# uber/petastorm

Measured on AMD Instinct MI355X. Metric: samples/sec/node (make_batch_reader->PyTorch DataLoader), imagenet config, higher is better.
Workload: dtype fp32; 1 GPU; model=ImageNetSchema(224x224x3 jpeg CompressedImageCodec + int32 label), global_batch=256, parallelism=dp1, prime_batches=0

## Files before the change

petastorm_amd/gpu/decoder.py:

```python

import os

import numpy as np
import torch

from petastorm_amd import ops
from petastorm_amd.codecs import (CompressedImageCodec, NdarrayCodec)

_ENC_PLAIN = 0
_ENC_PLAIN_DICT = 2
_ENC_RLE = 3
_ENC_DELTA_BINARY = 5
_ENC_DELTA_LENGTH_BA = 6
_ENC_DELTA_BA = 7
_ENC_RLE_DICT = 8
_ENC_BYTE_STREAM_SPLIT = 9
_PAGE_DATA_V1 = 0
_PAGE_DICT = 2
_PAGE_DATA_V2 = 3

_PHYS_TO_TORCH = {
    'INT32': (torch.int32, 4),
    'INT64': (torch.int64, 8),
    'FLOAT': (torch.float32, 4),
# ... 1268 lines not shown
                          status)
        self._check(status, 'png-inflate:' + field.name)
        out_bytes = row_bytes * heights
        out_off = np.zeros(n, dtype=np.int64)
        out_off[1:] = np.cumsum(out_bytes)[:-1]
        out = torch.empty(int(out_bytes.sum()) + _SLACK, dtype=torch.uint8,
                          device=dev)
        st2 = self._status(n)
        ext.png_unfilter_batch(raw, self._up(raw_off), out,
                               self._up(out_off),
                               self._up(meta['height']),
                               self._up(meta['row_bytes']),
                               self._up(meta['bpp']), st2)
        self._check(st2, 'png-unfilter:' + field.name)
        if len(set(widths.tolist())) != 1 or len(set(heights.tolist())) != 1 \
                or len(set(channels.tolist())) != 1 \
                or len(set(depth.tolist())) != 1:
            return None
        h, w, c, d = int(heights[0]), int(widths[0]), int(channels[0]), \
            int(depth[0])
        out = out[:int(out_bytes.sum())]
        if d == 16:
            ext.bswap16(out)
            t = out.view(torch.int16).view(n, h, w, c)
            t = t.to(torch.int32) & 0xFFFF
        else:
            t = out.view(n, h, w, c)
        return t.squeeze(-1) if c == 1 else t

    def decode_jpeg_column(self, col, field, fused_norm=None):
        if col.host_buf is None:
            return None
        ext = self._ext
        dev = self.device
        meta = col.jpeg_meta
        if meta is None:
            host_off = torch.from_numpy(col.host_val_off)
            host_len = col.val_len.cpu()
            meta = ext.jpeg_parse_batch(col.host_buf, host_off, host_len)
        n = col.n
        widths = meta['width'].numpy()
        heights = meta['height'].numpy()
        ncomp = meta['ncomp'].numpy()
        meta_dev = {}
        for k, v in meta.items():
            if not isinstance(v, torch.Tensor):
                meta_dev[k] = v
            elif k in ('seg_pos', 'seg_end'):
                meta_dev[k] = self._up(v)
            else:
                meta_dev[k] = self._up_cached(v)
        block_total = int(meta['block_total'])
        samp_total = int(meta['samp_total'])
        coef = torch.zeros(block_total * 64, dtype=torch.float32, device=dev)
        samples = torch.empty(samp_total, dtype=torch.uint8, device=dev)
        n_segs = int(meta['seg_img'].numel())
        uniform = (len(set(widths.tolist())) == 1 and
                   len(set(heights.tolist())) == 1 and
                   len(set(ncomp.tolist())) == 1)
        if fused_norm is not None and uniform and \
                self.device.type == 'cuda':
            H, W = int(heights[0]), int(widths[0])
            out_px = (widths.astype(np.int64) * heights * 3)
            out_off = np.zeros(n, dtype=np.int64)
            out_off[1:] = np.cumsum(out_px)[:-1]
            out = torch.empty(n, 3, H, W, dtype=torch.float32, device=dev)
            cache = getattr(self, '_fused_norm_cache', None)
            if cache is None:
                cache = self._fused_norm_cache = {}
            key = (tuple(fused_norm.mean), tuple(fused_norm.std))
            if key not in cache:
                mean_t = torch.tensor(fused_norm.mean, dtype=torch.float32,
                                      device=dev)
                inv_t = 1.0 / torch.tensor(fused_norm.std,
                                           dtype=torch.float32, device=dev)
                cache[key] = (mean_t, inv_t)
            mean_t, inv_t = cache[key]
            status = self._status(max(n_segs, 1))
            ext.jpeg_decode_fused_batch(
                col.device_buf, meta_dev, coef, samples, out.view(-1),
                self._up_cached(torch.from_numpy(out_off)), mean_t, inv_t,
                1.0 / fused_norm.scale_div, status)
            self._check(status, 'jpeg-fused:' + field.name)
            return out
        out_bytes = (widths.astype(np.int64) * heights *
                     np.where(ncomp == 3, 3, 1))
        out_off = np.zeros(n, dtype=np.int64)
        out_off[1:] = np.cumsum(out_bytes)[:-1]
        out = torch.empty(int(out_bytes.sum()), dtype=torch.uint8,
                          device=dev)
        status = self._status(max(n_segs, 1))
        ext.jpeg_decode_batch(col.device_buf, meta_dev, coef, samples, out,
                              self._up_cached(torch.from_numpy(out_off)),
                              status)
        self._check(status, 'jpeg:' + field.name)
        if uniform:
            c = 3 if ncomp[0] == 3 else 1
            t = out.view(n, int(heights[0]), int(widths[0]), c)
            return t if c == 3 else t.squeeze(-1)
        return None


def _widen_unsigned(t, np_dtype):
    if np_dtype == np.dtype(np.uint16):
        return t.to(torch.int32) & 0xFFFF
    if np_dtype == np.dtype(np.uint32):
        return t.to(torch.int64) & 0xFFFFFFFF
# ... 17 lines not shown
```

petastorm_amd/ops/csrc/ext.cpp:

```cpp
#include <torch/extension.h>

namespace psa {

void snappy_decompress_batch(torch::Tensor comp, torch::Tensor comp_start,
                             torch::Tensor comp_end, torch::Tensor out,
                             torch::Tensor out_offsets,
                             torch::Tensor out_len, torch::Tensor status);
void lz4_decompress_batch(torch::Tensor comp, torch::Tensor blk_start,
                          torch::Tensor blk_end, torch::Tensor out,
                          torch::Tensor out_offsets, torch::Tensor out_len,
                          torch::Tensor status);

void zstd_decompress_host(torch::Tensor src, torch::Tensor src_off,
                          torch::Tensor src_len, torch::Tensor dst,
                          torch::Tensor dst_off, torch::Tensor dst_len,
                          torch::Tensor status);

int64_t zstd_work_bytes();
void zstd_decompress_batch(torch::Tensor src, torch::Tensor src_off,
                           torch::Tensor src_len, torch::Tensor dst,
                           torch::Tensor dst_off, torch::Tensor dst_len,
                           torch::Tensor work, torch::Tensor status);

void rle_hybrid_decode_batch(torch::Tensor data, torch::Tensor start,
                             torch::Tensor end, torch::Tensor bit_width,
                             torch::Tensor n_values, torch::Tensor out_off,
                             torch::Tensor out, torch::Tensor status);
void byte_array_offsets_batch(torch::Tensor data, torch::Tensor start,
                              torch::Tensor end, torch::Tensor n_values,
                              torch::Tensor out_off, torch::Tensor val_off,
                              torch::Tensor val_len, torch::Tensor status);
void varlen_gather(torch::Tensor src, torch::Tensor src_off,
                   torch::Tensor lengths, torch::Tensor dst,
                   torch::Tensor dst_off);
void plain_fixed_decode_batch(torch::Tensor page_buf,
                              torch::Tensor payload_start,
                              torch::Tensor payload_end,
                              torch::Tensor n_values, torch::Tensor row0,
                              int64_t def_mode, int64_t esize,
                              int64_t fill_pattern, torch::Tensor def_buf,
                              torch::Tensor def_start, torch::Tensor def_len,
                              torch::Tensor out,
                              torch::Tensor valid_out, torch::Tensor status);
void npy_payload_offsets(torch::Tensor data, torch::Tensor val_off,
                         torch::Tensor val_len, torch::Tensor pay_off,
                         torch::Tensor pay_len, torch::Tensor status);
void nhwc_to_nchw_normalize(torch::Tensor in, torch::Tensor out,
                            torch::Tensor mean, torch::Tensor inv_std,
                            double scale);
py::dict jpeg_parse_batch(torch::Tensor buf, torch::Tensor val_off,
                          torch::Tensor val_len);
py::dict parquet_walk_pages(torch::Tensor buf, torch::Tensor chunk_off,
                            torch::Tensor chunk_len);
void inflate_batch(torch::Tensor src, torch::Tensor seg_off,
                   torch::Tensor seg_len, torch::Tensor seg_first,
                   torch::Tensor seg_count, torch::Tensor dst,
                   torch::Tensor dst_off, torch::Tensor dst_cap,
                   torch::Tensor produced, int64_t mode,
                   torch::Tensor status);
void png_unfilter_batch(torch::Tensor raw, torch::Tensor raw_off,
                        torch::Tensor out, torch::Tensor out_off,
                        torch::Tensor height, torch::Tensor row_bytes,
                        torch::Tensor bpp, torch::Tensor status);
void bswap16(torch::Tensor data);
py::dict png_parse_batch(torch::Tensor buf, torch::Tensor val_off,
                         torch::Tensor val_len);
py::dict byte_array_host_offsets(torch::Tensor buf, torch::Tensor val_start,
                                 torch::Tensor counts);
void jpeg_decode_batch(torch::Tensor data, py::dict meta, torch::Tensor coef,
                       torch::Tensor samples, torch::Tensor out,
                       torch::Tensor out_off, torch::Tensor status);
void delta_binary_packed_batch(torch::Tensor page_buf, torch::Tensor start,
                               torch::Tensor end, torch::Tensor n_values,
                               torch::Tensor out_off, torch::Tensor out,
                               int64_t esize, torch::Tensor status);
void delta_length_byte_array_batch(torch::Tensor page_buf,
                                   torch::Tensor start, torch::Tensor end,
                                   torch::Tensor n_values,
                                   torch::Tensor out_idx,
                                   torch::Tensor val_off,
                                   torch::Tensor val_len,
                                   torch::Tensor status);
void delta_byte_array_lengths_batch(torch::Tensor page_buf,
                                    torch::Tensor start, torch::Tensor end,
                                    torch::Tensor n_values,
                                    torch::Tensor out_idx,
                                    torch::Tensor pre, torch::Tensor sfx,
                                    torch::Tensor suf_data_pos,
                                    torch::Tensor status);
void delta_byte_array_reconstruct_batch(
    torch::Tensor page_buf, torch::Tensor n_values, torch::Tensor out_idx,
    torch::Tensor pre, torch::Tensor sfx, torch::Tensor suf_data_pos,
    torch::Tensor val_off, torch::Tensor out, torch::Tensor status);
void byte_stream_split_batch(torch::Tensor page_buf, torch::Tensor start,
                             torch::Tensor n_values, torch::Tensor out_off,
                             torch::Tensor out, int64_t esize);
void bool_unpack_batch(torch::Tensor page_buf, torch::Tensor start,
                       torch::Tensor n_values, torch::Tensor out_off,
                       torch::Tensor out);
void jpeg_decode_fused_batch(torch::Tensor data, py::dict meta,
                             torch::Tensor coef, torch::Tensor samples,
                             torch::Tensor out, torch::Tensor out_off,
                             torch::Tensor mean, torch::Tensor inv_std,
                             double scale, torch::Tensor status);

}

PYBIND11_MODULE(TORCH_EXTENSION_NAME, m) {
  m.doc() = "petastorm_amd MI355X (gfx950) decode kernels";
  m.def("snappy_decompress_batch", &psa::snappy_decompress_batch,
        "Batched snappy page decompression (wave-per-page)");
  m.def("lz4_decompress_batch", &psa::lz4_decompress_batch,
        "batch LZ4 block decompression, one wave per block");
  m.def("zstd_decompress_host", &psa::zstd_decompress_host,
        "batch ZSTD frame decompression on host threads (from-scratch "
        "RFC 8878 decoder, GIL released)");
  m.def("zstd_work_bytes", &psa::zstd_work_bytes,
        "per-frame device workspace size for zstd_decompress_batch");
  m.def("zstd_decompress_batch", &psa::zstd_decompress_batch,
        "batch ZSTD frame decompression on device (thread per frame)");
  m.def("rle_hybrid_decode_batch", &psa::rle_hybrid_decode_batch,
        "Parquet RLE/bit-packed hybrid decode (levels & dict indices)");
  m.def("byte_array_offsets_batch", &psa::byte_array_offsets_batch,
        "PLAIN byte-array page -> per-value (offset, length)");
  m.def("varlen_gather", &psa::varlen_gather,
        "Unaligned variable-length byte gather (funnel-shift copy)");
  m.def("plain_fixed_decode_batch", &psa::plain_fixed_decode_batch,
        "Fused PLAIN data-page decode: def levels + prefix scan + scatter");
  m.def("npy_payload_offsets", &psa::npy_payload_offsets,
        ".npy container -> payload (offset, length)");
  m.def("nhwc_to_nchw_normalize", &psa::nhwc_to_nchw_normalize,
        "Fused uint8 NHWC -> float NCHW normalize (LDS-tiled)");
  m.def("parquet_walk_pages", &psa::parquet_walk_pages,
        "Walk Parquet page headers (thrift compact) in a raw column chunk");
  m.def("inflate_batch", &psa::inflate_batch,
        "Batched DEFLATE inflate (zlib/raw), thread-per-stream");
  m.def("png_unfilter_batch", &psa::png_unfilter_batch,
        "PNG scanline unfilter (wave-per-image, bpp-lane chains)");
  m.def("bswap16", &psa::bswap16, "byte-swap 16-bit samples in place");
  m.def("png_parse_batch", &psa::png_parse_batch,
        "Host-side PNG container parse");
  m.def("byte_array_host_offsets", &psa::byte_array_host_offsets,
        "Host-side PLAIN byte-array offset scan");
  m.def("jpeg_parse_batch", &psa::jpeg_parse_batch,
        "Host-side JPEG header/segment parse");
  m.def("jpeg_decode_batch", &psa::jpeg_decode_batch,
        "GPU baseline JPEG decode (huffman/idct/color kernels)");
  m.def("delta_binary_packed_batch", &psa::delta_binary_packed_batch,
        "DELTA_BINARY_PACKED page decode (wave-per-page, shfl prefix scan)");
  m.def("delta_length_byte_array_batch",
        &psa::delta_length_byte_array_batch,
        "DELTA_LENGTH_BYTE_ARRAY page -> per-value (offset, length)");
  m.def("delta_byte_array_lengths_batch",
        &psa::delta_byte_array_lengths_batch,
        "DELTA_BYTE_ARRAY pass 1: prefix/suffix lengths");
  m.def("delta_byte_array_reconstruct_batch",
        &psa::delta_byte_array_reconstruct_batch,
        "DELTA_BYTE_ARRAY pass 2: materialize front-coded values");
  m.def("byte_stream_split_batch", &psa::byte_stream_split_batch,
        "BYTE_STREAM_SPLIT de-interleave");
  m.def("bool_unpack_batch", &psa::bool_unpack_batch,
        "PLAIN boolean bit-unpack");
  m.def("jpeg_decode_fused_batch", &psa::jpeg_decode_fused_batch,
        "JPEG decode with fused YCbCr->RGB + normalize + NCHW fp32 "
        "epilogue (skips the NHWC uint8 intermediate)");
}
```

petastorm_amd/ops/csrc/jpeg.hip:

```cpp
#include <hip/hip_runtime.h>
#include <torch/extension.h>
#include <c10/hip/HIPStream.h>
#include "common.h"

namespace psa {

__constant__ int ZIGZAG_NAT[64] = {
    0,  1,  8,  16, 9,  2,  3,  10, 17, 24, 32, 25, 18, 11, 4,  5,
    12, 19, 26, 33, 40, 48, 41, 34, 27, 20, 13, 6,  7,  14, 21, 28,
    35, 42, 49, 56, 57, 50, 43, 36, 29, 22, 15, 23, 30, 37, 44, 51,
    58, 59, 52, 45, 38, 31, 39, 46, 53, 60, 61, 54, 47, 55, 62, 63};

__constant__ float IDCT_B[8][8] = {
    {0.35355339f, 0.35355339f, 0.35355339f, 0.35355339f,
     0.35355339f, 0.35355339f, 0.35355339f, 0.35355339f},
    {0.49039264f, 0.41573481f, 0.27778512f, 0.09754516f,
     -0.09754516f, -0.27778512f, -0.41573481f, -0.49039264f},
    {0.46193977f, 0.19134172f, -0.19134172f, -0.46193977f,
     -0.46193977f, -0.19134172f, 0.19134172f, 0.46193977f},
    {0.41573481f, -0.09754516f, -0.49039264f, -0.27778512f,
     0.27778512f, 0.49039264f, 0.09754516f, -0.41573481f},
    {0.35355339f, -0.35355339f, -0.35355339f, 0.35355339f,
     0.35355339f, -0.35355339f, -0.35355339f, 0.35355339f},
    {0.27778512f, -0.49039264f, 0.09754516f, 0.41573481f,
     -0.41573481f, -0.09754516f, 0.49039264f, -0.27778512f},
    {0.19134172f, -0.46193977f, 0.46193977f, -0.19134172f,
     -0.19134172f, 0.46193977f, -0.46193977f, 0.19134172f},
    {0.09754516f, -0.27778512f, 0.41573481f, -0.49039264f,
     0.49039264f, -0.41573481f, 0.27778512f, -0.09754516f}};

struct JpegTables {
  const int32_t* lut;
  const int32_t* maxcode;
  const int32_t* mincode;
  const int32_t* valptr;
  const uint8_t* huffval;
  const float* qtabs;
};

struct JpegGeom {
  const int32_t* comp_h;
  const int32_t* comp_v;
  const int32_t* comp_q;
  const int32_t* comp_dc;
  const int32_t* comp_ac;
  const int64_t* samp_off;
  const int32_t* samp_stride;
  const int32_t* mcus_x;
  const int32_t* mcus_y;
  const int32_t* ncomp;
  const int32_t* width;
  const int32_t* height;
  const int64_t* img_block0;
  const int32_t* bpm;
  const int32_t* kmap;
};


struct BitReader {
  const uint8_t* p;
  int64_t pos, end;
  uint64_t buf;
  int cnt;
  uint32_t sw0, sw1;
  int64_t spos;
  int scount;

  __device__ void init(const uint8_t* data, int64_t lo, int64_t hi) {
    p = data; pos = lo; end = hi; buf = 0; cnt = 0; scount = 0; spos = 0;
  }
  __device__ __forceinline__ void fill() {
    while (cnt <= 32) {
      if (pos + 4 <= end) {
        uint32_t w;
        if (scount > 0 && spos == pos) {
          w = sw0;
          sw0 = sw1;
          spos += 4;
          --scount;
        } else {
          scount = 0;
          w = (uint32_t)p[pos] | ((uint32_t)p[pos + 1] << 8) |
              ((uint32_t)p[pos + 2] << 16) | ((uint32_t)p[pos + 3] << 24);
          if (pos + 12 <= end) {
            sw0 = (uint32_t)p[pos + 4] | ((uint32_t)p[pos + 5] << 8) |
                  ((uint32_t)p[pos + 6] << 16) |
                  ((uint32_t)p[pos + 7] << 24);
            sw1 = (uint32_t)p[pos + 8] | ((uint32_t)p[pos + 9] << 8) |
                  ((uint32_t)p[pos + 10] << 16) |
                  ((uint32_t)p[pos + 11] << 24);
            spos = pos + 4;
            scount = 2;
          } else if (pos + 8 <= end) {
            sw0 = (uint32_t)p[pos + 4] | ((uint32_t)p[pos + 5] << 8) |
                  ((uint32_t)p[pos + 6] << 16) |
                  ((uint32_t)p[pos + 7] << 24);
            spos = pos + 4;
            scount = 1;
          }
        }
        uint32_t inv = ~w;
        if (!((inv - 0x01010101u) & ~inv & 0x80808080u)) {
          uint32_t be = __builtin_bswap32(w);
          buf |= (uint64_t)be << (32 - cnt);
          cnt += 32;
          pos += 4;
          continue;
        }
      }
      uint8_t b = 0;
      if (pos < end) {
        b = p[pos];
        if (b == 0xFF) {
          if (pos + 1 < end && p[pos + 1] == 0x00) {
            pos += 2;
          } else {
            pos = end;
            b = 0;
          }
        } else {
          pos += 1;
        }
      } else {
        buf |= 0;
        cnt += 8;
        continue;
      }
      buf |= (uint64_t)b << (56 - cnt);
      cnt += 8;
    }
  }
  __device__ __forceinline__ uint32_t peek(int n) {
    return (uint32_t)(buf >> (64 - n));
  }
  __device__ __forceinline__ void consume(int n) {
    buf <<= n;
    cnt -= n;
  }
};

__device__ __forceinline__ int huff_decode(BitReader& br,
                                           const JpegTables& t, int tid) {
  br.fill();
  uint32_t look = br.peek(8);
  int32_t hit = t.lut[tid * 256 + look];
  if (hit >= 0) {
    br.consume(hit >> 16);
    return hit & 0xFF;
  }
  for (int l = 9; l <= 16; ++l) {
    int32_t code = (int32_t)br.peek(l);
    int32_t mc = t.maxcode[tid * 18 + l];
    if (mc >= 0 && code <= mc) {
      br.consume(l);
      int idx = t.valptr[tid * 18 + l] + code - t.mincode[tid * 18 + l];
      return t.huffval[tid * 256 + idx];
    }
  }
  return -1;
}

__device__ __forceinline__ int receive_extend(BitReader& br, int s) {
  br.fill();
  int v = (int)br.peek(s);
  br.consume(s);
  if (v < (1 << (s - 1))) v += (-1 << s) + 1;
  return v;
}

template <bool NT>
__device__ __forceinline__ int decode_block(BitReader& br,
                                            const JpegTables& tabs,
                                            const float* __restrict__ q,
                                            int dc_t, int ac_t,
                                            float* __restrict__ out,
                                            int& pred) {
  int t = huff_decode(br, tabs, dc_t);
  if (t < 0 || t > 15) return 10;
  int diff = t ? receive_extend(br, t) : 0;
  pred += diff;
  if (NT) __builtin_nontemporal_store((float)pred * q[0], out);
  else out[0] = (float)pred * q[0];
  int kk = 1;
  while (kk < 64) {
    int rs = huff_decode(br, tabs, ac_t);
    if (rs < 0) return 11;
    int r = rs >> 4, sz = rs & 15;
    if (sz == 0) {
      if (r != 15) break;
      kk += 16;
    } else {
      kk += r;
      if (kk > 63) return 12;
      int v = receive_extend(br, sz);
      if (NT) __builtin_nontemporal_store((float)v * q[kk],
                                          out + ZIGZAG_NAT[kk]);
      else out[ZIGZAG_NAT[kk]] = (float)v * q[kk];
      ++kk;
    }
  }
  return 0;
}

template <bool NT>
__global__ void jpeg_huffman_kernel(
    const uint8_t* __restrict__ data, JpegTables tabs, JpegGeom g,
    const int32_t* __restrict__ seg_img, const int64_t* __restrict__ seg_pos,
    const int64_t* __restrict__ seg_end, const int32_t* __restrict__ seg_mcu0,
    const int32_t* __restrict__ seg_nmcu, float* __restrict__ coef,
    int32_t* __restrict__ status, int n_segs) {
  int s = blockIdx.x * blockDim.x + threadIdx.x;
  if (s >= n_segs) return;
  const int img = seg_img[s];
  const int bpm = g.bpm[img];
  const int ncomp = g.ncomp[img];

  BitReader br;
  br.init(data, seg_pos[s], seg_end[s]);

  const float* q0 = tabs.qtabs + (int64_t)g.comp_q[img * 3 + 0] * 64;
  const int dc0 = g.comp_dc[img * 3 + 0], ac0 = g.comp_ac[img * 3 + 0];
  const int rep0 = g.comp_h[img * 3 + 0] * g.comp_v[img * 3 + 0];
  const float* q1 = q0;
  const float* q2 = q0;
  int dc1 = 0, ac1 = 0, dc2 = 0, ac2 = 0;
  if (ncomp == 3) {
    q1 = tabs.qtabs + (int64_t)g.comp_q[img * 3 + 1] * 64;
    dc1 = g.comp_dc[img * 3 + 1];
    ac1 = g.comp_ac[img * 3 + 1];
    q2 = tabs.qtabs + (int64_t)g.comp_q[img * 3 + 2] * 64;
    dc2 = g.comp_dc[img * 3 + 2];
    ac2 = g.comp_ac[img * 3 + 2];
  }

  int pred0 = 0, pred1 = 0, pred2 = 0;
  const int mcu0 = seg_mcu0[s];
  const int nmcu = seg_nmcu[s];
  const int64_t blk0 = g.img_block0[img];

  for (int m = 0; m < nmcu; ++m) {
    float* mcu_out = coef + (blk0 + (int64_t)(mcu0 + m) * bpm) * 64;
    int rc = 0;
    for (int r = 0; r < rep0 && !rc; ++r, mcu_out += 64)
      rc = decode_block<NT>(br, tabs, q0, dc0, ac0, mcu_out, pred0);
    if (!rc && ncomp == 3) {
      rc = decode_block<NT>(br, tabs, q1, dc1, ac1, mcu_out, pred1);
      mcu_out += 64;
      if (!rc)
        rc = decode_block<NT>(br, tabs, q2, dc2, ac2, mcu_out, pred2);
    }
    if (rc) { status[s] = rc; return; }
  }
}


__global__ void jpeg_idct_kernel(const float* __restrict__ coef,
                                 JpegGeom g, uint8_t* __restrict__ samples,
                                 int n_imgs, int64_t block_total) {
  int64_t b = (int64_t)blockIdx.x * blockDim.x + threadIdx.x;
  if (b >= block_total) return;
  int lo = 0, hi = n_imgs - 1;
  while (lo < hi) {
    int mid = (lo + hi + 1) >> 1;
    if (g.img_block0[mid] <= b) lo = mid; else hi = mid - 1;
  }
  const int img = lo;
  const int bpm = g.bpm[img];
  const int64_t r = b - g.img_block0[img];
  const int m = (int)(r / bpm);
  const int k = (int)(r % bpm);
  const int km = g.kmap[img * 8 + k];
  const int c = km >> 8, v = (km >> 4) & 15, h = km & 15;
  const int mx = m % g.mcus_x[img];
  const int my = m / g.mcus_x[img];
  const int stride = g.samp_stride[img * 3 + c];
  uint8_t* dst = samples + g.samp_off[img * 3 + c] +
                 ((int64_t)(my * g.comp_v[img * 3 + c] + v) * 8) * stride +
                 (int64_t)(mx * g.comp_h[img * 3 + c] + h) * 8;

  const float* C = coef + b * 64;
  float tmp[64];
#pragma unroll
  for (int vv = 0; vv < 8; ++vv) {
#pragma unroll
    for (int x = 0; x < 8; ++x) {
      float acc = 0.f;
#pragma unroll
      for (int u = 0; u < 8; ++u) acc += C[vv * 8 + u] * IDCT_B[u][x];
      tmp[vv * 8 + x] = acc;
    }
  }
#pragma unroll
  for (int y = 0; y < 8; ++y) {
    uint8_t row[8];
#pragma unroll
    for (int x = 0; x < 8; ++x) {
      float acc = 0.f;
#pragma unroll
      for (int vv = 0; vv < 8; ++vv) acc += tmp[vv * 8 + x] * IDCT_B[vv][y];
      int pix = __float2int_rn(acc) + 128;
      row[x] = (uint8_t)min(255, max(0, pix));
    }
    *(uint64_t*)(dst + (int64_t)y * stride) = *(const uint64_t*)row;
  }
// ... 147 lines not shown
      rpix[k] = ((float)min(255, max(0, rv)) * scale - m0) * s0;
      gpix[k] = ((float)min(255, max(0, gv)) * scale - m1) * s1;
      bpix[k] = ((float)min(255, max(0, bv)) * scale - m2) * s2;
    }
    float* dr = dst + pix0;
    float* dg = dst + plane + pix0;
    float* db = dst + 2 * plane + pix0;
    if (cnt == 4 && ((pix0 & 3) == 0)) {
      *(float4*)dr = make_float4(rpix[0], rpix[1], rpix[2], rpix[3]);
      *(float4*)dg = make_float4(gpix[0], gpix[1], gpix[2], gpix[3]);
      *(float4*)db = make_float4(bpix[0], bpix[1], bpix[2], bpix[3]);
    } else {
      for (int k = 0; k < cnt; ++k) {
        dr[k] = rpix[k];
        dg[k] = gpix[k];
        db[k] = bpix[k];
      }
    }
  }
}


static JpegTables make_tables(const py::dict& d) {
  JpegTables t;
  t.lut = d["lut"].cast<torch::Tensor>().data_ptr<int32_t>();
  t.maxcode = d["maxcode"].cast<torch::Tensor>().data_ptr<int32_t>();
  t.mincode = d["mincode"].cast<torch::Tensor>().data_ptr<int32_t>();
  t.valptr = d["valptr"].cast<torch::Tensor>().data_ptr<int32_t>();
  t.huffval = d["huffval"].cast<torch::Tensor>().data_ptr<uint8_t>();
  t.qtabs = d["qtabs"].cast<torch::Tensor>().data_ptr<float>();
  return t;
}

static JpegGeom make_geom(const py::dict& d) {
  JpegGeom g;
  g.comp_h = d["comp_h"].cast<torch::Tensor>().data_ptr<int32_t>();
  g.comp_v = d["comp_v"].cast<torch::Tensor>().data_ptr<int32_t>();
  g.comp_q = d["comp_q"].cast<torch::Tensor>().data_ptr<int32_t>();
  g.comp_dc = d["comp_dc"].cast<torch::Tensor>().data_ptr<int32_t>();
  g.comp_ac = d["comp_ac"].cast<torch::Tensor>().data_ptr<int32_t>();
  g.samp_off = d["samp_off"].cast<torch::Tensor>().data_ptr<int64_t>();
  g.samp_stride = d["samp_stride"].cast<torch::Tensor>().data_ptr<int32_t>();
  g.mcus_x = d["mcus_x"].cast<torch::Tensor>().data_ptr<int32_t>();
  g.mcus_y = d["mcus_y"].cast<torch::Tensor>().data_ptr<int32_t>();
  g.ncomp = d["ncomp"].cast<torch::Tensor>().data_ptr<int32_t>();
  g.width = d["width"].cast<torch::Tensor>().data_ptr<int32_t>();
  g.height = d["height"].cast<torch::Tensor>().data_ptr<int32_t>();
  g.img_block0 = d["img_block0"].cast<torch::Tensor>().data_ptr<int64_t>();
  g.bpm = d["bpm"].cast<torch::Tensor>().data_ptr<int32_t>();
  g.kmap = d["kmap"].cast<torch::Tensor>().data_ptr<int32_t>();
  return g;
}

void jpeg_decode_batch(torch::Tensor data, py::dict meta, torch::Tensor coef,
                       torch::Tensor samples, torch::Tensor out,
                       torch::Tensor out_off, torch::Tensor status) {
  TORCH_CHECK(data.is_cuda() && coef.is_cuda() && samples.is_cuda() &&
              out.is_cuda());
  JpegTables tabs = make_tables(meta);
  JpegGeom g = make_geom(meta);
  auto seg_img = meta["seg_img"].cast<torch::Tensor>();
  auto seg_pos = meta["seg_pos"].cast<torch::Tensor>();
  auto seg_end = meta["seg_end"].cast<torch::Tensor>();
  auto seg_mcu0 = meta["seg_mcu0"].cast<torch::Tensor>();
  auto seg_nmcu = meta["seg_nmcu"].cast<torch::Tensor>();
  int n_segs = (int)seg_img.numel();
  int n_imgs = (int)meta["width"].cast<torch::Tensor>().numel();
  int64_t block_total = coef.numel() / 64;
  hipStream_t stream = c10::hip::getCurrentHIPStream();

  static const bool use_nt = [] {
    const char* e = getenv("PSA_JPEG_NT");
    return e && e[0] == '1';
  }();
  if (use_nt)
    hipLaunchKernelGGL(jpeg_huffman_kernel<true>,
                       dim3((n_segs + 63) / 64), dim3(64), 0, stream,
                       data.data_ptr<uint8_t>(), tabs, g,
                       seg_img.data_ptr<int32_t>(),
                       seg_pos.data_ptr<int64_t>(),
                       seg_end.data_ptr<int64_t>(),
                       seg_mcu0.data_ptr<int32_t>(),
                       seg_nmcu.data_ptr<int32_t>(), coef.data_ptr<float>(),
                       status.data_ptr<int32_t>(), n_segs);
  else
    hipLaunchKernelGGL(jpeg_huffman_kernel<false>,
                       dim3((n_segs + 63) / 64), dim3(64), 0, stream,
                       data.data_ptr<uint8_t>(), tabs, g,
                       seg_img.data_ptr<int32_t>(),
                       seg_pos.data_ptr<int64_t>(),
                       seg_end.data_ptr<int64_t>(),
                       seg_mcu0.data_ptr<int32_t>(),
                       seg_nmcu.data_ptr<int32_t>(), coef.data_ptr<float>(),
                       status.data_ptr<int32_t>(), n_segs);

  hipLaunchKernelGGL(jpeg_idct_kernel,
                     dim3((unsigned)((block_total + 255) / 256)), dim3(256),
                     0, stream, coef.data_ptr<float>(), g,
                     samples.data_ptr<uint8_t>(), n_imgs, block_total);

  int64_t avg_bytes = n_imgs > 0 ? out.numel() / n_imgs : 0;
  int64_t est_blocks = (avg_bytes / 12 + 255) / 256;
  int grid_x = (int)std::min<int64_t>(std::max<int64_t>(est_blocks, 1), 2048);
  hipLaunchKernelGGL(jpeg_color_kernel, dim3(grid_x, n_imgs), dim3(256), 0,
                     stream, samples.data_ptr<uint8_t>(), g,
                     out.data_ptr<uint8_t>(), out_off.data_ptr<int64_t>(),
                     n_imgs);
}

void jpeg_decode_fused_batch(torch::Tensor data, py::dict meta,
                             torch::Tensor coef, torch::Tensor samples,
                             torch::Tensor out, torch::Tensor out_off,
                             torch::Tensor mean, torch::Tensor inv_std,
                             double scale, torch::Tensor status) {
  TORCH_CHECK(data.is_cuda() && coef.is_cuda() && samples.is_cuda() &&
              out.is_cuda() && out.scalar_type() == torch::kFloat32);
  TORCH_CHECK(mean.is_cuda() && inv_std.is_cuda() &&
              mean.numel() == 3 && inv_std.numel() == 3);
  JpegTables tabs = make_tables(meta);
  JpegGeom g = make_geom(meta);
  auto seg_img = meta["seg_img"].cast<torch::Tensor>();
  auto seg_pos = meta["seg_pos"].cast<torch::Tensor>();
  auto seg_end = meta["seg_end"].cast<torch::Tensor>();
  auto seg_mcu0 = meta["seg_mcu0"].cast<torch::Tensor>();
  auto seg_nmcu = meta["seg_nmcu"].cast<torch::Tensor>();
  int n_segs = (int)seg_img.numel();
  int n_imgs = (int)meta["width"].cast<torch::Tensor>().numel();
  int64_t block_total = coef.numel() / 64;
  hipStream_t stream = c10::hip::getCurrentHIPStream();

  static const bool use_nt = [] {
    const char* e = getenv("PSA_JPEG_NT");
    return e && e[0] == '1';
  }();
  if (use_nt)
    hipLaunchKernelGGL(jpeg_huffman_kernel<true>,
                       dim3((n_segs + 63) / 64), dim3(64), 0, stream,
                       data.data_ptr<uint8_t>(), tabs, g,
                       seg_img.data_ptr<int32_t>(),
                       seg_pos.data_ptr<int64_t>(),
                       seg_end.data_ptr<int64_t>(),
                       seg_mcu0.data_ptr<int32_t>(),
                       seg_nmcu.data_ptr<int32_t>(), coef.data_ptr<float>(),
                       status.data_ptr<int32_t>(), n_segs);
  else
    hipLaunchKernelGGL(jpeg_huffman_kernel<false>,
                       dim3((n_segs + 63) / 64), dim3(64), 0, stream,
                       data.data_ptr<uint8_t>(), tabs, g,
                       seg_img.data_ptr<int32_t>(),
                       seg_pos.data_ptr<int64_t>(),
                       seg_end.data_ptr<int64_t>(),
                       seg_mcu0.data_ptr<int32_t>(),
                       seg_nmcu.data_ptr<int32_t>(), coef.data_ptr<float>(),
                       status.data_ptr<int32_t>(), n_segs);

  hipLaunchKernelGGL(jpeg_idct_kernel,
                     dim3((unsigned)((block_total + 255) / 256)), dim3(256),
                     0, stream, coef.data_ptr<float>(), g,
                     samples.data_ptr<uint8_t>(), n_imgs, block_total);

  int64_t avg_px = n_imgs > 0 ? out.numel() / (3 * n_imgs) : 0;
  int64_t est_blocks = (avg_px / 4 + 255) / 256;
  int grid_x = (int)std::min<int64_t>(std::max<int64_t>(est_blocks, 1), 2048);
  hipLaunchKernelGGL(jpeg_color_norm_kernel, dim3(grid_x, n_imgs), dim3(256),
                     0, stream, samples.data_ptr<uint8_t>(), g,
                     out.data_ptr<float>(), out_off.data_ptr<int64_t>(),
                     mean.data_ptr<float>(), inv_std.data_ptr<float>(),
                     (float)scale, n_imgs);
}

}
```

Baseline: 559,900 samples/sec.

## Stage JPEG Huffman tables and bitstream in LDS with tiled coefficient stores

```diff
diff --git a/petastorm_amd/gpu/decoder.py b/petastorm_amd/gpu/decoder.py
--- a/petastorm_amd/gpu/decoder.py
+++ b/petastorm_amd/gpu/decoder.py
@@ -1344,7 +1344,7 @@
                 meta_dev[k] = self._up_cached(v)
         block_total = int(meta['block_total'])
         samp_total = int(meta['samp_total'])
-        coef = torch.zeros(block_total * 64, dtype=torch.float32, device=dev)
+        coef = torch.empty(block_total * 64, dtype=torch.float32, device=dev)
         samples = torch.empty(samp_total, dtype=torch.uint8, device=dev)
         n_segs = int(meta['seg_img'].numel())
         uniform = (len(set(widths.tolist())) == 1 and
diff --git a/petastorm_amd/ops/csrc/ext.cpp b/petastorm_amd/ops/csrc/ext.cpp
--- a/petastorm_amd/ops/csrc/ext.cpp
+++ b/petastorm_amd/ops/csrc/ext.cpp
@@ -69,7 +69,8 @@
                                  torch::Tensor counts);
 void jpeg_decode_batch(torch::Tensor data, py::dict meta, torch::Tensor coef,
                        torch::Tensor samples, torch::Tensor out,
-                       torch::Tensor out_off, torch::Tensor status);
+                       torch::Tensor out_off, torch::Tensor status,
+                       int64_t staging);
 void delta_binary_packed_batch(torch::Tensor page_buf, torch::Tensor start,
                                torch::Tensor end, torch::Tensor n_values,
                                torch::Tensor out_off, torch::Tensor out,
@@ -102,7 +103,8 @@
                              torch::Tensor coef, torch::Tensor samples,
                              torch::Tensor out, torch::Tensor out_off,
                              torch::Tensor mean, torch::Tensor inv_std,
-                             double scale, torch::Tensor status);
+                             double scale, torch::Tensor status,
+                             int64_t staging);
 
 }
 
@@ -145,7 +147,10 @@
   m.def("jpeg_parse_batch", &psa::jpeg_parse_batch,
         "Host-side JPEG header/segment parse");
   m.def("jpeg_decode_batch", &psa::jpeg_decode_batch,
-        "GPU baseline JPEG decode (huffman/idct/color kernels)");
+        "GPU baseline JPEG decode (huffman/idct/color kernels)",
+        py::arg("data"), py::arg("meta"), py::arg("coef"),
+        py::arg("samples"), py::arg("out"), py::arg("out_off"),
+        py::arg("status"), py::arg("staging") = -1);
   m.def("delta_binary_packed_batch", &psa::delta_binary_packed_batch,
         "DELTA_BINARY_PACKED page decode (wave-per-page, shfl prefix scan)");
   m.def("delta_length_byte_array_batch",
@@ -163,5 +168,9 @@
         "PLAIN boolean bit-unpack");
   m.def("jpeg_decode_fused_batch", &psa::jpeg_decode_fused_batch,
         "JPEG decode with fused YCbCr->RGB + normalize + NCHW fp32 "
-        "epilogue (skips the NHWC uint8 intermediate)");
+        "epilogue (skips the NHWC uint8 intermediate)",
+        py::arg("data"), py::arg("meta"), py::arg("coef"),
+        py::arg("samples"), py::arg("out"), py::arg("out_off"),
+        py::arg("mean"), py::arg("inv_std"), py::arg("scale"),
+        py::arg("status"), py::arg("staging") = -1);
 }
diff --git a/petastorm_amd/ops/csrc/jpeg.hip b/petastorm_amd/ops/csrc/jpeg.hip
--- a/petastorm_amd/ops/csrc/jpeg.hip
+++ b/petastorm_amd/ops/csrc/jpeg.hip
@@ -57,47 +57,82 @@
 };
 
 
+constexpr int kLdsHuff = 4;
+constexpr int kLdsQ = 4;
+constexpr int kWinBytes = 8192;
+
+typedef float f32x4 __attribute__((ext_vector_type(4)));
+
+__constant__ uint8_t NAT_ZIGZAG[64] = {
+    0,  1,  5,  6,  14, 15, 27, 28, 2,  4,  7,  13, 16, 26, 29, 42,
+    3,  8,  12, 17, 25, 30, 41, 43, 9,  11, 18, 24, 31, 40, 44, 53,
+    10, 19, 23, 32, 39, 45, 52, 54, 20, 22, 33, 38, 46, 51, 55, 60,
+    21, 34, 37, 47, 50, 56, 59, 61, 35, 36, 48, 49, 57, 58, 62, 63};
+
+struct GlobalBytes {
+  typedef int64_t pos_t;
+  static constexpr bool kPrefetch = true;
+  const uint8_t* p;
+  __device__ __forceinline__ uint32_t byte(pos_t i) const { return p[i]; }
+  __device__ __forceinline__ uint32_t word(pos_t i) const {
+    return (uint32_t)p[i] | ((uint32_t)p[i + 1] << 8) |
+           ((uint32_t)p[i + 2] << 16) | ((uint32_t)p[i + 3] << 24);
+  }
+};
+
+struct LdsBytes {
+  typedef int pos_t;
+  static constexpr bool kPrefetch = false;
+  const uint32_t* w;
+  __device__ __forceinline__ uint32_t byte(pos_t i) const {
+    return (w[i >> 2] >> ((i & 3) * 8)) & 0xFFu;
+  }
+  __device__ __forceinline__ uint32_t word(pos_t i) const {
+    const uint64_t two = ((uint64_t)w[(i >> 2) + 1] << 32) | w[i >> 2];
+    return (uint32_t)(two >> ((i & 3) * 8));
+  }
+};
+
+template <class Src>
 struct BitReader {
-  const uint8_t* p;
-  int64_t pos, end;
+  typedef typename Src::pos_t pos_t;
+  Src src;
+  pos_t pos, end;
   uint64_t buf;
   int cnt;
   uint32_t sw0, sw1;
-  int64_t spos;
+  pos_t spos;
   int scount;
 
-  __device__ void init(const uint8_t* data, int64_t lo, int64_t hi) {
-    p = data; pos = lo; end = hi; buf = 0; cnt = 0; scount = 0; spos = 0;
+  __device__ void init(Src s, pos_t lo, pos_t hi) {
+    src = s; pos = lo; end = hi; buf = 0; cnt = 0; scount = 0; spos = 0;
   }
   __device__ __forceinline__ void fill() {
     while (cnt <= 32) {
       if (pos + 4 <= end) {
         uint32_t w;
-        if (scount > 0 && spos == pos) {
-          w = sw0;
-          sw0 = sw1;
-          spos += 4;
-          --scount;
+        if constexpr (Src::kPrefetch) {
+          if (scount > 0 && spos == pos) {
+            w = sw0;
+            sw0 = sw1;
+            spos += 4;
+            --scount;
+          } else {
+            scount = 0;
+            w = src.word(pos);
+            if (pos + 12 <= end) {
+              sw0 = src.word(pos + 4);
+              sw1 = src.word(pos + 8);
+              spos = pos + 4;
+              scount = 2;
+            } else if (pos + 8 <= end) {
+              sw0 = src.word(pos + 4);
+              spos = pos + 4;
+              scount = 1;
+            }
+          }
         } else {
-          scount = 0;
-          w = (uint32_t)p[pos] | ((uint32_t)p[pos + 1] << 8) |
-              ((uint32_t)p[pos + 2] << 16) | ((uint32_t)p[pos + 3] << 24);
-          if (pos + 12 <= end) {
-            sw0 = (uint32_t)p[pos + 4] | ((uint32_t)p[pos + 5] << 8) |
-                  ((uint32_t)p[pos + 6] << 16) |
-                  ((uint32_t)p[pos + 7] << 24);
-            sw1 = (uint32_t)p[pos + 8] | ((uint32_t)p[pos + 9] << 8) |
-                  ((uint32_t)p[pos + 10] << 16) |
-                  ((uint32_t)p[pos + 11] << 24);
-            spos = pos + 4;
-            scount = 2;
-          } else if (pos + 8 <= end) {
-            sw0 = (uint32_t)p[pos + 4] | ((uint32_t)p[pos + 5] << 8) |
-                  ((uint32_t)p[pos + 6] << 16) |
-                  ((uint32_t)p[pos + 7] << 24);
-            spos = pos + 4;
-            scount = 1;
-          }
+          w = src.word(pos);
         }
         uint32_t inv = ~w;
         if (!((inv - 0x01010101u) & ~inv & 0x80808080u)) {
@@ -108,11 +143,11 @@
           continue;
         }
       }
-      uint8_t b = 0;
+      uint32_t b = 0;
       if (pos < end) {
-        b = p[pos];
+        b = src.byte(pos);
         if (b == 0xFF) {
-          if (pos + 1 < end && p[pos + 1] == 0x00) {
+          if (pos + 1 < end && src.byte(pos + 1) == 0x00) {
             pos += 2;
           } else {
             pos = end;
@@ -122,7 +157,6 @@
           pos += 1;
         }
       } else {
-        buf |= 0;
         cnt += 8;
         continue;
       }
@@ -139,15 +173,46 @@
   }
 };
 
-__device__ __forceinline__ int huff_decode(BitReader& br,
-                                           const JpegTables& t, int tid) {
+template <bool TAB>
+struct HuffTabs {
+  JpegTables t;
+  const uint16_t* lut16;
+  const int32_t* maxcode;
+  const int32_t* valoff;
+  const uint8_t* huffval;
+  const uint8_t* zz;
+};
+
+template <class Src, bool TAB>
+__device__ __forceinline__ int huff_decode(BitReader<Src>& br,
+                                           const HuffTabs<TAB>& ht, int tid) {
   br.fill();
   uint32_t look = br.peek(8);
-  int32_t hit = t.lut[tid * 256 + look];
-  if (hit >= 0) {
-    br.consume(hit >> 16);
-    return hit & 0xFF;
-  }
+  if constexpr (TAB) {
+    uint32_t e = ht.lut16[tid * 256 + look];
+    if (e != 0xFFFFu) {
+      br.consume(e >> 8);
+      return e & 0xFF;
+    }
+    const uint32_t look16 = br.peek(16);
+    int len = 0;
+#pragma unroll
+    for (int l = 16; l >= 9; --l) {
+      const int32_t mc = ht.maxcode[tid * 18 + l];
+      if (mc >= 0 && (int32_t)(look16 >> (16 - l)) <= mc) len = l;
+    }
+    if (len == 0) return -1;
+    br.consume(len);
+    const int idx = ht.valoff[tid * 18 + len] + (int)(look16 >> (16 - len));
+    return ht.huffval[tid * 256 + (idx & 255)];
+  } else {
+    int32_t hit = ht.t.lut[tid * 256 + look];
+    if (hit >= 0) {
+      br.consume(hit >> 16);
+      return hit & 0xFF;
+    }
+  }
+  const JpegTables& t = ht.t;
   for (int l = 9; l <= 16; ++l) {
     int32_t code = (int32_t)br.peek(l);
     int32_t mc = t.maxcode[tid * 18 + l];
@@ -160,30 +225,32 @@
   return -1;
 }
 
-__device__ __forceinline__ int receive_extend(BitReader& br, int s) {
-  br.fill();
+template <class Src>
+__device__ __forceinline__ int receive_extend(BitReader<Src>& br, int s) {
   int v = (int)br.peek(s);
   br.consume(s);
   if (v < (1 << (s - 1))) v += (-1 << s) + 1;
   return v;
 }
 
-template <bool NT>
-__device__ __forceinline__ int decode_block(BitReader& br,
-                                            const JpegTables& tabs,
-                                            const float* __restrict__ q,
-                                            int dc_t, int ac_t,
-                                            float* __restrict__ out,
-                                            int& pred) {
-  int t = huff_decode(br, tabs, dc_t);
+__device__ __forceinline__ int tile_swz(int b) {
+  return ((b & 15) << 2) | (((b >> 4) & 1) << 1);
+}
+
+template <class Src, bool TAB>
+__device__ __forceinline__ int decode_block(BitReader<Src>& br,
+                                            const HuffTabs<TAB>& ht,
+                                            int dc_t, int ac_t, float q_dc,
+                                            int16_t* blk, int swz,
+                                            int& pred, float& dc_out) {
+  int t = huff_decode(br, ht, dc_t);
   if (t < 0 || t > 15) return 10;
   int diff = t ? receive_extend(br, t) : 0;
   pred += diff;
-  if (NT) __builtin_nontemporal_store((float)pred * q[0], out);
-  else out[0] = (float)pred * q[0];
+  dc_out = (float)pred * q_dc;
   int kk = 1;
   while (kk < 64) {
-    int rs = huff_decode(br, tabs, ac_t);
+    int rs = huff_decode(br, ht, ac_t);
     if (rs < 0) return 11;
     int r = rs >> 4, sz = rs & 15;
     if (sz == 0) {
@@ -193,63 +260,243 @@
       kk += r;
       if (kk > 63) return 12;
       int v = receive_extend(br, sz);
-      if (NT) __builtin_nontemporal_store((float)v * q[kk],
-                                          out + ZIGZAG_NAT[kk]);
-      else out[ZIGZAG_NAT[kk]] = (float)v * q[kk];
+      int nat;
+      if constexpr (TAB) nat = ht.zz[kk];
+      else nat = ZIGZAG_NAT[kk];
+      blk[nat ^ swz] = (int16_t)v;
       ++kk;
     }
   }
   return 0;
 }
 
-template <bool NT>
-__global__ void jpeg_huffman_kernel(
-    const uint8_t* __restrict__ data, JpegTables tabs, JpegGeom g,
+template <bool TAB>
+__device__ __forceinline__ void drain_tile(uint64_t* tile64, const float* qn,
+                                           const float* gq, int lane,
+                                           uint64_t have_mask, int gblk,
+                                           int qt, float dcv,
+                                           float* __restrict__ coef,
+                                           bool nt) {
+  const int sub = lane >> 4, p = lane & 15;
+#pragma unroll 1
+  for (int j = 0; j < 16; ++j) {
+    if (((have_mask >> (4 * j)) & 0xF) == 0) continue;
+    const int b = 4 * j + sub;
+    const int gb = __shfl(gblk, b);
+    const int qb = __shfl(qt, b);
+    const float db = __shfl(dcv, b);
+    const int slot = b * 16 + (p ^ (b & 15));
+    const uint64_t raw = tile64[slot];
+    tile64[slot] = 0;
+    uint32_t lo = (uint32_t)raw, hi = (uint32_t)(raw >> 32);
+    if ((b >> 4) & 1) { uint32_t x = lo; lo = hi; hi = x; }
+    const int v0 = (int16_t)(lo & 0xFFFF), v1 = (int16_t)(lo >> 16);
+    const int v2 = (int16_t)(hi & 0xFFFF), v3 = (int16_t)(hi >> 16);
+    f32x4 q;
+    if constexpr (TAB) {
+      q = *(const f32x4*)(qn + qb * 64 + 4 * p);
+    } else {
+      const float* qg = gq + (int64_t)qb * 64;
+      q.x = qg[NAT_ZIGZAG[4 * p + 0]];
+      q.y = qg[NAT_ZIGZAG[4 * p + 1]];
+      q.z = qg[NAT_ZIGZAG[4 * p + 2]];
+      q.w = qg[NAT_ZIGZAG[4 * p + 3]];
+    }
+    f32x4 o;
+    o.x = (p == 0) ? db : (float)v0 * q.x;
+    o.y = (float)v1 * q.y;
+    o.z = (float)v2 * q.z;
+    o.w = (float)v3 * q.w;
+    if (gb >= 0) {
+      f32x4* dst = (f32x4*)(coef + (int64_t)gb * 64 + 4 * p);
+      if (nt) __builtin_nontemporal_store(o, dst);
+      else *dst = o;
+    }
+  }
+}
+
+template <class Src, bool TAB>
+__device__ __forceinline__ void run_steps(
+    Src src, typename Src::pos_t lo, typename Src::pos_t hi,
+    const HuffTabs<TAB>& ht, int max_nblk, int16_t* tile,
+    const float* qn, float* __restrict__ coef, int32_t* status_slot,
+    bool nt, int lane,
+    int nblk, int blk_base, int bpm, int cpack,
+    int dc0, int ac0, int qt0, float qdc0,
+    int dc1, int ac1, int qt1, float qdc1,
+    int dc2, int ac2, int qt2, float qdc2) {
+  BitReader<Src> br;
+  br.init(src, lo, hi);
+  int pred0 = 0, pred1 = 0, pred2 = 0;
+  int rc = 0, k = 0;
+  int16_t* blk = tile + lane * 64;
+  const int swz = tile_swz(lane);
+  for (int step = 0; step < max_nblk; ++step) {
+    const bool have = step < nblk;
+    const int c = (cpack >> (2 * k)) & 3;
+    float dcv = 0.f;
+    if (have && !rc) {
+      const int dc_t = c == 0 ? dc0 : c == 1 ? dc1 : dc2;
+      const int ac_t = c == 0 ? ac0 : c == 1 ? ac1 : ac2;
+      const float q_dc = c == 0 ? qdc0 : c == 1 ? qdc1 : qdc2;
+      int pred = c == 0 ? pred0 : c == 1 ? pred1 : pred2;
+      rc = decode_block(br, ht, dc_t, ac_t, q_dc, blk, swz, pred, dcv);
+      pred0 = c == 0 ? pred : pred0;
+      pred1 = c == 1 ? pred : pred1;
+      pred2 = c == 2 ? pred : pred2;
+      if (rc) *status_slot = rc;
+    }
+    const int qt = c == 0 ? qt0 : c == 1 ? qt1 : qt2;
+    if (have && ++k == bpm) k = 0;
+    __syncthreads();
+    drain_tile<TAB>((uint64_t*)tile, qn, ht.t.qtabs, lane, __ballot(have),
+                    have ? blk_base + step : -1, qt, dcv, coef, nt);
+    __syncthreads();
+  }
+}
+
+__device__ __forceinline__ int wave_max_i32(int v) {
+  for (int o = 32; o; o >>= 1) v = max(v, __shfl_xor(v, o));
+  return v;
+}
+__device__ __forceinline__ int64_t wave_max_i64(int64_t v) {
+  for (int o = 32; o; o >>= 1) {
+    int64_t u = __shfl_xor((long long)v, o);
+    v = u > v ? u : v;
+  }
+  return v;
+}
+
+template <bool TAB, bool BS>
+__global__ void __launch_bounds__(64) jpeg_huffman_kernel(
+    const uint8_t* __restrict__ data, int64_t data_len, JpegTables tabs,
+    int n_huff, int n_q, JpegGeom g,
     const int32_t* __restrict__ seg_img, const int64_t* __restrict__ seg_pos,
     const int64_t* __restrict__ seg_end, const int32_t* __restrict__ seg_mcu0,
     const int32_t* __restrict__ seg_nmcu, float* __restrict__ coef,
-    int32_t* __restrict__ status, int n_segs) {
-  int s = blockIdx.x * blockDim.x + threadIdx.x;
-  if (s >= n_segs) return;
-  const int img = seg_img[s];
-  const int bpm = g.bpm[img];
-  const int ncomp = g.ncomp[img];
-
-  BitReader br;
-  br.init(data, seg_pos[s], seg_end[s]);
-
-  const float* q0 = tabs.qtabs + (int64_t)g.comp_q[img * 3 + 0] * 64;
-  const int dc0 = g.comp_dc[img * 3 + 0], ac0 = g.comp_ac[img * 3 + 0];
-  const int rep0 = g.comp_h[img * 3 + 0] * g.comp_v[img * 3 + 0];
-  const float* q1 = q0;
-  const float* q2 = q0;
-  int dc1 = 0, ac1 = 0, dc2 = 0, ac2 = 0;
-  if (ncomp == 3) {
-    q1 = tabs.qtabs + (int64_t)g.comp_q[img * 3 + 1] * 64;
-    dc1 = g.comp_dc[img * 3 + 1];
-    ac1 = g.comp_ac[img * 3 + 1];
-    q2 = tabs.qtabs + (int64_t)g.comp_q[img * 3 + 2] * 64;
-    dc2 = g.comp_dc[img * 3 + 2];
-    ac2 = g.comp_ac[img * 3 + 2];
-  }
-
-  int pred0 = 0, pred1 = 0, pred2 = 0;
-  const int mcu0 = seg_mcu0[s];
-  const int nmcu = seg_nmcu[s];
-  const int64_t blk0 = g.img_block0[img];
-
-  for (int m = 0; m < nmcu; ++m) {
-    float* mcu_out = coef + (blk0 + (int64_t)(mcu0 + m) * bpm) * 64;
-    int rc = 0;
-    for (int r = 0; r < rep0 && !rc; ++r, mcu_out += 64)
-      rc = decode_block<NT>(br, tabs, q0, dc0, ac0, mcu_out, pred0);
-    if (!rc && ncomp == 3) {
-      rc = decode_block<NT>(br, tabs, q1, dc1, ac1, mcu_out, pred1);
-      mcu_out += 64;
-      if (!rc)
-        rc = decode_block<NT>(br, tabs, q2, dc2, ac2, mcu_out, pred2);
-    }
-    if (rc) { status[s] = rc; return; }
+    int32_t* __restrict__ status, int n_segs, bool nt) {
+  __shared__ __attribute__((aligned(16))) int16_t tile[64 * 64];
+  __shared__ __attribute__((aligned(16))) float qn[TAB ? kLdsQ * 64 : 4];
+  __shared__ uint16_t lut16[TAB ? kLdsHuff * 256 : 2];
+  __shared__ int32_t smax[TAB ? kLdsHuff * 18 : 1];
+  __shared__ int32_t svoff[TAB ? kLdsHuff * 18 : 1];
+  __shared__ uint32_t shval[TAB ? kLdsHuff * 64 : 1];
+  __shared__ uint8_t zz[TAB ? 64 : 4];
+  __shared__ __attribute__((aligned(16)))
+      uint32_t win[BS ? kWinBytes / 4 + 4 : 4];
+
+  const int lane = threadIdx.x;
+  const int s = blockIdx.x * 64 + lane;
+  const bool valid = s < n_segs;
+
+  for (int i = lane; i < 64 * 64 / 4; i += 64) ((uint64_t*)tile)[i] = 0;
+  if constexpr (TAB) {
+    for (int i = lane; i < n_huff * 256; i += 64) {
+      const int32_t h = tabs.lut[i];
+      lut16[i] = h < 0 ? (uint16_t)0xFFFF
+                       : (uint16_t)(((h >> 16) << 8) | (h & 0xFF));
+    }
+    for (int i = lane; i < n_huff * 18; i += 64) {
+      smax[i] = tabs.maxcode[i];
+      svoff[i] = tabs.valptr[i] - tabs.mincode[i];
+    }
+    for (int i = lane; i < n_huff * 64; i += 64)
+      shval[i] = ((const uint32_t*)tabs.huffval)[i];
+    zz[lane] = (uint8_t)ZIGZAG_NAT[lane];
+    for (int i = lane; i < n_q * 64; i += 64)
+      qn[(i & ~63) + ZIGZAG_NAT[i & 63]] = tabs.qtabs[i];
+  }
+
+  int nblk = 0, blk_base = 0, bpm = 1, cpack = 0;
+  int dc0 = 0, ac0 = 0, qt0 = 0, dc1 = 0, ac1 = 0, qt1 = 0;
+  int dc2 = 0, ac2 = 0, qt2 = 0;
+  float qdc0 = 0.f, qdc1 = 0.f, qdc2 = 0.f;
+  int64_t lo = 0, hi = 0;
+  if (valid) {
+    const int img = seg_img[s];
+    const int ncomp = g.ncomp[img];
+    bpm = g.bpm[img];
+    lo = seg_pos[s];
+    hi = seg_end[s];
+    qt0 = g.comp_q[img * 3 + 0];
+    dc0 = g.comp_dc[img * 3 + 0];
+    ac0 = g.comp_ac[img * 3 + 0];
+    qdc0 = tabs.qtabs[(int64_t)qt0 * 64];
+    if (ncomp == 3) {
+      qt1 = g.comp_q[img * 3 + 1];
+      dc1 = g.comp_dc[img * 3 + 1];
+      ac1 = g.comp_ac[img * 3 + 1];
+      qdc1 = tabs.qtabs[(int64_t)qt1 * 64];
+      qt2 = g.comp_q[img * 3 + 2];
+      dc2 = g.comp_dc[img * 3 + 2];
+      ac2 = g.comp_ac[img * 3 + 2];
+      qdc2 = tabs.qtabs[(int64_t)qt2 * 64];
+    }
+    for (int k = 0; k < bpm; ++k)
+      cpack |= ((g.kmap[img * 8 + k] >> 8) & 3) << (2 * k);
+    nblk = max(seg_nmcu[s], 0) * bpm;
+    blk_base = (int)(g.img_block0[img] + (int64_t)seg_mcu0[s] * bpm);
+  }
+  const int max_nblk = __builtin_amdgcn_readfirstlane(wave_max_i32(nblk));
+
+  bool staged = false;
+  int64_t win_base = 0;
+  if constexpr (BS) {
+    const int64_t wlo = -wave_max_i64(valid ? -lo : -INT64_MAX);
+    const int64_t whi = wave_max_i64(valid ? hi : -INT64_MAX);
+    win_base = wlo & ~(int64_t)15;
+    staged = whi >= wlo && whi - win_base <= kWinBytes;
+    if (staged) {
+      const int nchunk = (int)((whi - win_base + 15) >> 4);
+      for (int c = lane; c < nchunk; c += 64) {
+        const int64_t off = win_base + 16 * (int64_t)c;
+        uint4 v;
+        if (off + 16 <= data_len) {
+          v = *(const uint4*)(data + off);
+        } else {
+          uint32_t w0 = 0, w1 = 0, w2 = 0, w3 = 0;
+#pragma unroll
+          for (int e = 0; e < 4; ++e) {
+            const int sh = 8 * e;
+            if (off + e < data_len) w0 |= (uint32_t)data[off + e] << sh;
+            if (off + 4 + e < data_len)
+              w1 |= (uint32_t)data[off + 4 + e] << sh;
+            if (off + 8 + e < data_len)
+              w2 |= (uint32_t)data[off + 8 + e] << sh;
+            if (off + 12 + e < data_len)
+              w3 |= (uint32_t)data[off + 12 + e] << sh;
+          }
+          v = make_uint4(w0, w1, w2, w3);
+        }
+        ((uint4*)win)[c] = v;
+      }
+    }
+  }
+  __syncthreads();
+
+  HuffTabs<TAB> ht;
+  ht.t = tabs;
+  ht.lut16 = lut16;
+  ht.maxcode = smax;
+  ht.valoff = svoff;
+  ht.huffval = (const uint8_t*)shval;
+  ht.zz = zz;
+  int32_t* status_slot = status + (valid ? s : 0);
+  if (staged) {
+    LdsBytes src;
+    src.w = win;
+    run_steps<LdsBytes, TAB>(src, (int)(lo - win_base), (int)(hi - win_base),
+                             ht, max_nblk, tile, qn, coef, status_slot,
+                             nt, lane, nblk, blk_base, bpm, cpack,
+                             dc0, ac0, qt0, qdc0, dc1, ac1, qt1, qdc1,
+                             dc2, ac2, qt2, qdc2);
+  } else {
+    GlobalBytes src;
+    src.p = data;
+    run_steps<GlobalBytes, TAB>(src, lo, hi, ht, max_nblk, tile, qn, coef,
+                                status_slot, nt, lane, nblk, blk_base, bpm,
+                                cpack, dc0, ac0, qt0, qdc0, dc1, ac1, qt1,
+                                qdc1, dc2, ac2, qt2, qdc2);
   }
 }
 
@@ -503,52 +750,89 @@
   return g;
 }
 
-void jpeg_decode_batch(torch::Tensor data, py::dict meta, torch::Tensor coef,
-                       torch::Tensor samples, torch::Tensor out,
-                       torch::Tensor out_off, torch::Tensor status) {
-  TORCH_CHECK(data.is_cuda() && coef.is_cuda() && samples.is_cuda() &&
-              out.is_cuda());
+static int resolve_staging(int64_t staging) {
+  if (staging >= 0) {
+    TORCH_CHECK(staging <= 3, "jpeg staging switch must be -1..3");
+    return (int)staging;
+  }
+  static const int auto_mode = [] {
+    const char* e = getenv("PSA_JPEG_STAGING");
+    return (e && e[0] >= '0' && e[0] <= '3' && !e[1]) ? e[0] - '0' : 3;
+  }();
+  return auto_mode;
+}
+
+static int launch_huffman_idct(const torch::Tensor& data,
+                               const py::dict& meta, const JpegGeom& g,
+                               const torch::Tensor& coef,
+                               const torch::Tensor& samples,
+                               const torch::Tensor& status, int64_t staging,
+                               hipStream_t stream) {
   JpegTables tabs = make_tables(meta);
-  JpegGeom g = make_geom(meta);
   auto seg_img = meta["seg_img"].cast<torch::Tensor>();
   auto seg_pos = meta["seg_pos"].cast<torch::Tensor>();
   auto seg_end = meta["seg_end"].cast<torch::Tensor>();
   auto seg_mcu0 = meta["seg_mcu0"].cast<torch::Tensor>();
   auto seg_nmcu = meta["seg_nmcu"].cast<torch::Tensor>();
-  int n_segs = (int)seg_img.numel();
-  int n_imgs = (int)meta["width"].cast<torch::Tensor>().numel();
-  int64_t block_total = coef.numel() / 64;
-  hipStream_t stream = c10::hip::getCurrentHIPStream();
+  const int n_segs = (int)seg_img.numel();
+  const int n_imgs = (int)meta["width"].cast<torch::Tensor>().numel();
+  const int64_t block_total = meta["block_total"].cast<int64_t>();
+  const int n_huff = (int)meta["lut"].cast<torch::Tensor>().size(0);
+  const int n_q = (int)meta["qtabs"].cast<torch::Tensor>().size(0);
+  TORCH_CHECK(coef.scalar_type() == torch::kFloat32 &&
+              coef.numel() >= block_total * 64,
+              "coef must hold block_total*64 floats");
+  TORCH_CHECK(block_total < (int64_t)1 << 31);
+  TORCH_CHECK(((uintptr_t)coef.data_ptr<float>() & 15) == 0,
+              "coef must be 16-byte aligned");
+  TORCH_CHECK(status.numel() >= n_segs);
+
+  int mode = resolve_staging(staging);
+  if (n_huff > kLdsHuff || n_q > kLdsQ) mode &= ~1;
+  if ((uintptr_t)tabs.huffval & 3) mode &= ~1;
+  if ((uintptr_t)data.data_ptr<uint8_t>() & 15) mode &= ~2;
 
   static const bool use_nt = [] {
     const char* e = getenv("PSA_JPEG_NT");
     return e && e[0] == '1';
   }();
-  if (use_nt)
-    hipLaunchKernelGGL(jpeg_huffman_kernel<true>,
-                       dim3((n_segs + 63) / 64), dim3(64), 0, stream,
-                       data.data_ptr<uint8_t>(), tabs, g,
-                       seg_img.data_ptr<int32_t>(),
+
+  auto huffman = [&](auto kernel) {
+    hipLaunchKernelGGL(kernel, dim3((n_segs + 63) / 64), dim3(64), 0, stream,
+                       data.data_ptr<uint8_t>(), (int64_t)data.numel(), tabs,
+                       n_huff, n_q, g, seg_img.data_ptr<int32_t>(),
                        seg_pos.data_ptr<int64_t>(),
                        seg_end.data_ptr<int64_t>(),
                        seg_mcu0.data_ptr<int32_t>(),
                        seg_nmcu.data_ptr<int32_t>(), coef.data_ptr<float>(),
-                       status.data_ptr<int32_t>(), n_segs);
-  else
-    hipLaunchKernelGGL(jpeg_huffman_kernel<false>,
-                       dim3((n_segs + 63) / 64), dim3(64), 0, stream,
-                       data.data_ptr<uint8_t>(), tabs, g,
-                       seg_img.data_ptr<int32_t>(),
-                       seg_pos.data_ptr<int64_t>(),
-                       seg_end.data_ptr<int64_t>(),
-                       seg_mcu0.data_ptr<int32_t>(),
-                       seg_nmcu.data_ptr<int32_t>(), coef.data_ptr<float>(),
-                       status.data_ptr<int32_t>(), n_segs);
-
-  hipLaunchKernelGGL(jpeg_idct_kernel,
-                     dim3((unsigned)((block_total + 255) / 256)), dim3(256),
-                     0, stream, coef.data_ptr<float>(), g,
-                     samples.data_ptr<uint8_t>(), n_imgs, block_total);
+                       status.data_ptr<int32_t>(), n_segs, use_nt);
+  };
+  if (n_segs > 0) {
+    switch (mode) {
+      case 0: huffman(jpeg_huffman_kernel<false, false>); break;
+      case 1: huffman(jpeg_huffman_kernel<true, false>); break;
+      case 2: huffman(jpeg_huffman_kernel<false, true>); break;
+      default: huffman(jpeg_huffman_kernel<true, true>); break;
+    }
+  }
+  if (block_total > 0)
+    hipLaunchKernelGGL(jpeg_idct_kernel,
+                       dim3((unsigned)((block_total + 255) / 256)), dim3(256),
+                       0, stream, coef.data_ptr<float>(), g,
+                       samples.data_ptr<uint8_t>(), n_imgs, block_total);
+  return n_imgs;
+}
+
+void jpeg_decode_batch(torch::Tensor data, py::dict meta, torch::Tensor coef,
+                       torch::Tensor samples, torch::Tensor out,
+                       torch::Tensor out_off, torch::Tensor status,
+                       int64_t staging) {
+  TORCH_CHECK(data.is_cuda() && coef.is_cuda() && samples.is_cuda() &&
+              out.is_cuda());
+  JpegGeom g = make_geom(meta);
+  hipStream_t stream = c10::hip::getCurrentHIPStream();
+  const int n_imgs = launch_huffman_idct(data, meta, g, coef, samples, status,
+                                         staging, stream);
 
   int64_t avg_bytes = n_imgs > 0 ? out.numel() / n_imgs : 0;
   int64_t est_blocks = (avg_bytes / 12 + 255) / 256;
@@ -563,52 +847,16 @@
                              torch::Tensor coef, torch::Tensor samples,
                              torch::Tensor out, torch::Tensor out_off,
                              torch::Tensor mean, torch::Tensor inv_std,
-                             double scale, torch::Tensor status) {
+                             double scale, torch::Tensor status,
+                             int64_t staging) {
   TORCH_CHECK(data.is_cuda() && coef.is_cuda() && samples.is_cuda() &&
               out.is_cuda() && out.scalar_type() == torch::kFloat32);
   TORCH_CHECK(mean.is_cuda() && inv_std.is_cuda() &&
               mean.numel() == 3 && inv_std.numel() == 3);
-  JpegTables tabs = make_tables(meta);
   JpegGeom g = make_geom(meta);
-  auto seg_img = meta["seg_img"].cast<torch::Tensor>();
-  auto seg_pos = meta["seg_pos"].cast<torch::Tensor>();
-  auto seg_end = meta["seg_end"].cast<torch::Tensor>();
-  auto seg_mcu0 = meta["seg_mcu0"].cast<torch::Tensor>();
-  auto seg_nmcu = meta["seg_nmcu"].cast<torch::Tensor>();
-  int n_segs = (int)seg_img.numel();
-  int n_imgs = (int)meta["width"].cast<torch::Tensor>().numel();
-  int64_t block_total = coef.numel() / 64;
   hipStream_t stream = c10::hip::getCurrentHIPStream();
-
-  static const bool use_nt = [] {
-    const char* e = getenv("PSA_JPEG_NT");
-    return e && e[0] == '1';
-  }();
-  if (use_nt)
-    hipLaunchKernelGGL(jpeg_huffman_kernel<true>,
-                       dim3((n_segs + 63) / 64), dim3(64), 0, stream,
-                       data.data_ptr<uint8_t>(), tabs, g,
-                       seg_img.data_ptr<int32_t>(),
-                       seg_pos.data_ptr<int64_t>(),
-                       seg_end.data_ptr<int64_t>(),
-                       seg_mcu0.data_ptr<int32_t>(),
-                       seg_nmcu.data_ptr<int32_t>(), coef.data_ptr<float>(),
-                       status.data_ptr<int32_t>(), n_segs);
-  else
-    hipLaunchKernelGGL(jpeg_huffman_kernel<false>,
-                       dim3((n_segs + 63) / 64), dim3(64), 0, stream,
-                       data.data_ptr<uint8_t>(), tabs, g,
-                       seg_img.data_ptr<int32_t>(),
-                       seg_pos.data_ptr<int64_t>(),
-                       seg_end.data_ptr<int64_t>(),
-                       seg_mcu0.data_ptr<int32_t>(),
-                       seg_nmcu.data_ptr<int32_t>(), coef.data_ptr<float>(),
-                       status.data_ptr<int32_t>(), n_segs);
-
-  hipLaunchKernelGGL(jpeg_idct_kernel,
-                     dim3((unsigned)((block_total + 255) / 256)), dim3(256),
-                     0, stream, coef.data_ptr<float>(), g,
-                     samples.data_ptr<uint8_t>(), n_imgs, block_total);
+  const int n_imgs = launch_huffman_idct(data, meta, g, coef, samples, status,
+                                         staging, stream);
 
   int64_t avg_px = n_imgs > 0 ? out.numel() / (3 * n_imgs) : 0;
   int64_t est_blocks = (avg_px / 4 + 255) / 256;
```

Result: faster. 613,000 samples/sec (median of 6 runs) (+9.5%).
